# theo2021/OnDA

Measured on AMD Instinct MI355X. Metric: adaptation-step images/sec (fwd+bwd+proto) 512x1024 bs=4, higher is better.
Workload: dtype f32 (f16x2 split emulation); 1 GPU; hybrid_switch adaptation step (step + update_ema), 1024x512, bs=4 per micro-batch, 1 micro-batch(es) per GPU and optimizer step, dynamic branch, DeepLabV2-ResNet50 ProDA head, random-init weights; global_batch=4, parallelism=dp1, branch=dynamic, micro_batches_per_gpu=1, inputs=resident in HBM

## Files before the change

### onda_amd/csrc/conv_l2.hip

```cpp
#include "conv_common.h"

namespace {

typedef _Float16 f16x8 __attribute__((ext_vector_type(8)));
typedef _Float16 f16x2 __attribute__((ext_vector_type(2)));
typedef _Float16 f16x4 __attribute__((ext_vector_type(4)));
typedef float f32x2 __attribute__((ext_vector_type(2)));
typedef unsigned int u32x2 __attribute__((ext_vector_type(2)));
typedef unsigned int u32x4 __attribute__((ext_vector_type(4)));
typedef int i32x4 __attribute__((ext_vector_type(4)));

#define ZZ(i, jj) (((i) & 1) ? 3 - (jj) : (jj))

constexpr float LIMB2_SCALE = ONDA_LIMB2_SCALE, LIMB2_UNSCALE = 1.f / ONDA_LIMB2_SCALE;

#ifndef ONDA_NT_OUT
#define ONDA_NT_OUT 1
#endif
constexpr int NT_AUX = ONDA_NT_OUT ? 2 : 0;
template <class T>
__device__ __forceinline__ void store_out(T* p, T v) {
  if constexpr (ONDA_NT_OUT) __builtin_nontemporal_store(v, p); else *p = v;
}
constexpr unsigned OOB = 0x80000000u;
// ... 29 lines not shown
  const bool ok = (unsigned)hi < (unsigned)c.Hi && (unsigned)wi < (unsigned)c.Wi;
  return ok ? (unsigned)(((p.bH + hi) * c.Wi + wi) * c.ldx) * 4u + chunk16 : 0x80000000u;
}

struct Scale2 {
  float s, inv;
};
__device__ __forceinline__ Scale2 scale_from(float m);
__device__ __forceinline__ Scale2 scale_of(const float* __restrict__ amax) { return scale_from(amax_read(amax)); }
__device__ __forceinline__ Scale2 scale_from(const float m) {
  int e = 0;
  if (m > 0.f && m < 3.0e38f) {
    int ex;
    frexpf(m, &ex);
    e = 15 - ex;
    e = e > 100 ? 100 : (e < -100 ? -100 : e);
  }
  return Scale2{ldexpf(1.f, e), ldexpf(1.f, -e)};
}

__device__ __forceinline__ unsigned cvt2h(float lo, float hi) {
  return __builtin_bit_cast(unsigned, __builtin_convertvector(f32x2{lo, hi}, f16x2));
}
__device__ __forceinline__ f32x2 unpack2h(unsigned p) {
  return __builtin_convertvector(__builtin_bit_cast(f16x2, p), f32x2);
}

__global__ __launch_bounds__(256) void split_h2_kernel(const float* __restrict__ x, long long rows, int C, int ldx,
                                                       _Float16* __restrict__ dst, int ldo, long long plane,
                                                       const float* __restrict__ amax) {
  const float s = scale_of(amax).s;
  const int c8 = C >> 3;
  const long long n = rows * c8;
  for (long long e = (long long)blockIdx.x * 256 + threadIdx.x; e < n; e += (long long)gridDim.x * 256) {
    const long long row = e / c8;
    const int ch = (int)(e - row * c8) * 8;
    const f32x4 v0 = *reinterpret_cast<const f32x4*>(x + row * ldx + ch) * s;
    const f32x4 v1 = *reinterpret_cast<const f32x4*>(x + row * ldx + ch + 4) * s;
    u32x4 l1, l2;
#pragma unroll
    for (int h = 0; h < 4; ++h) {
      const float a = h < 2 ? v0[2 * h] : v1[2 * h - 4], b = h < 2 ? v0[2 * h + 1] : v1[2 * h - 3];
      const unsigned p = cvt2h(a, b);
      const f32x2 f = unpack2h(p);
      l1[h] = p;
      l2[h] = cvt2h((a - f[0]) * LIMB2_SCALE, (b - f[1]) * LIMB2_SCALE);
    }
    _Float16* o = dst + limb_at((size_t)row, ch, ldo);
    *reinterpret_cast<u32x4*>(o) = l1;
    *reinterpret_cast<u32x4*>(o + LIMB2_OFS) = l2;
  }
}

__global__ __launch_bounds__(256) void stem_im2col_l2_kernel(const float* __restrict__ x, _Float16* __restrict__ dst,
                                                             long long plane, int B, int H, int W, int Ho, int Wo, int Kp,
                                                             const float* __restrict__ amax) {
  const float sc = scale_of(amax).s;
  const int k8 = Kp >> 3;
  const long long n = (long long)B * Ho * Wo * k8;
  for (long long e = (long long)blockIdx.x * 256 + threadIdx.x; e < n; e += (long long)gridDim.x * 256) {
    const long long m = e / k8;
    const int k0 = (int)(e - m * k8) * 8;
    const int wo = (int)(m % Wo);
    const long long tq = m / Wo;
    const int ho = (int)(tq % Ho), b = (int)(tq / Ho);
    float v[8];
#pragma unroll
    for (int j = 0; j < 8; ++j) {
      const int k = k0 + j;
      float val = 0.f;
      if (k < 147) {
        const int tap = k / 3, cc = k - tap * 3;
        const int r = tap / 7, t7 = tap - r * 7;
        const int hi = ho * 2 - 3 + r, wi = wo * 2 - 3 + t7;
        if ((unsigned)hi < (unsigned)H && (unsigned)wi < (unsigned)W) val = x[(((size_t)b * 3 + cc) * H + hi) * W + wi];
      }
      v[j] = val * sc;
    }
    u32x4 l1, l2;
#pragma unroll
    for (int h = 0; h < 4; ++h) {
      const unsigned pk = cvt2h(v[2 * h], v[2 * h + 1]);
      const f32x2 f = unpack2h(pk);
      l1[h] = pk;
      l2[h] = cvt2h((v[2 * h] - f[0]) * LIMB2_SCALE, (v[2 * h + 1] - f[1]) * LIMB2_SCALE);
    }
    _Float16* o = dst + limb_at((size_t)m, k0, Kp);
    *reinterpret_cast<u32x4*>(o) = l1;
    *reinterpret_cast<u32x4*>(o + LIMB2_OFS) = l2;
  }
}

#define ONDA_SWAP4(INSN, A, B)                                                                                          \
  asm volatile("s_nop 1\n\t" INSN " %0, %4\n\t" INSN " %1, %5\n\t" INSN " %2, %6\n\t" INSN " %3, %7\n\ts_nop 0"         \
               : "+v"(A[0]), "+v"(A[1]), "+v"(A[2]), "+v"(A[3]), "+v"(B[0]), "+v"(B[1]), "+v"(B[2]), "+v"(B[3]))
__device__ __forceinline__ void rows_reduce4(float& s1, float& s2, float& mn, float& mx) {
#if defined(__HIP_DEVICE_COMPILE__)
  float A[4] = {s1, s2, mn, mx}, B[4] = {s1, s2, mn, mx};
  ONDA_SWAP4("v_permlane16_swap_b32", A, B);
  float C[4] = {A[0] + B[0], A[1] + B[1], fminf(A[2], B[2]), fmaxf(A[3], B[3])};
  float D[4] = {C[0], C[1], C[2], C[3]};
  ONDA_SWAP4("v_permlane32_swap_b32", C, D);
  s1 = C[0] + D[0];
  s2 = C[1] + D[1];
  mn = fminf(C[2], D[2]);
  mx = fmaxf(C[3], D[3]);
#endif
}

template <int WM, int WN, bool COUNTED = false, bool AFFINE = true>
__device__ __forceinline__ void l2_epilogue(const ConvK& a, const f32x4 (&acc)[4][4], unsigned char* scratch, int tile_m, int m0,
                                            int n0, int wm, int wn, int lane, float ua, float ub, unsigned y_bytes = 0) {
  constexpr int BN = 64 * WN, NW = WM * WN, NT = NW * 64;
  constexpr int TRS = 68;
  const OndaConv& c = a.c;
  const int t = threadIdx.x, wave = t >> 6;
  unsigned long long* est = a.stamps != nullptr && t == 0 ? a.stamps + (size_t)blockIdx.x * 32 + 24 : nullptr;
  if (est) est[0] = __builtin_amdgcn_s_memtime();
  float* red = reinterpret_cast<float*>(scratch + NW * (16 * TRS * 4));
  const int SR = a.stats_rows;
  if (a.stats != nullptr) {
#pragma unroll
    for (int jn = 0; jn < 4; ++jn) {
      float s1 = 0.f, s2 = 0.f, mn = 3.0e38f, mxv = -3.0e38f;
#pragma unroll
      for (int i = 0; i < 4; ++i)
#pragma unroll
        for (int e = 0; e < 4; ++e) {
          const float v = acc[i][jn][e];
          s1 += v;
          s2 += v * v;
          mn = fminf(mn, v);
          mxv = fmaxf(mxv, v);
        }
      rows_reduce4(s1, s2, mn, mxv);
      if (lane < 16) {
        const int col = (wn * 4 + jn) * 16 + lane;
        red[(wm * BN + col) * 4 + 0] = (s1 * ua) * ub;
        red[(wm * BN + col) * 4 + 1] = (((s2 * ua) * ub) * ua) * ub;
        red[(wm * BN + col) * 4 + 2] = (mn * ua) * ub;
        red[(wm * BN + col) * 4 + 3] = (mxv * ua) * ub;
      }
// ... 1688 lines not shown
    }
    if (!late && nlive > 0) __builtin_amdgcn_s_barrier();
  }

#pragma unroll
  for (int i = 0; i < 4; ++i)
#pragma unroll
    for (int j = 0; j < 4; ++j) acc[i][j] = ((acc[i][j] + accx[i][j] * LIMB2_UNSCALE) * unscale_a) * unscale_b;
  if (stp) stp[2] = __builtin_amdgcn_s_memtime();
  __syncthreads();
  float* tr = reinterpret_cast<float*>(lds + (t >> 6) * 4096);
  const int cl = (lane & 15) * 4, rl = lane >> 4;
  const int cc = c0 + wn * 64 + cl;
#pragma unroll
  for (int i = 0; i < 4; ++i) {
#pragma unroll
    for (int jn = 0; jn < 4; ++jn)
#pragma unroll
      for (int e = 0; e < 4; ++e) tr[(4 * (lane >> 4) + e) * 64 + jn * 16 + (lane & 15)] = acc[i][jn][e];
    __builtin_amdgcn_wave_barrier();
#pragma unroll
    for (int r = 0; r < 4; ++r) {
      const int row = 4 * r + rl;
      const f32x4 v = *reinterpret_cast<const f32x4*>(tr + row * 64 + cl);
      const int n = n0 + (wm * 4 + i) * 16 + row;
      if (n < c.Cout && cc < c.Cin) *reinterpret_cast<f32x4*>(a.slabs + (((size_t)ks * c.Cout + n) * a.taps + tap) * c.Cin + cc) = v;
    }
    __builtin_amdgcn_wave_barrier();
  }
  if (stp) stp[3] = __builtin_amdgcn_s_memtime();
}

}

extern "C" {

int onda_split_h2(const float* x, int64_t rows, int C, int ldx, void* dst, int ldo, int64_t plane, const float* amax,
                  onda_stream_t s) {
  (void)plane;
  ONDA_REQUIRE(x && dst && amax && rows > 0 && C > 0 && C % 8 == 0 && ldx >= C && ldx % 4 == 0 && ldo >= C && ldo % 32 == 0);
  if (!ONDA_ALIGNED16(x) || !ONDA_ALIGNED16(dst)) return ONDA_EALIGN;
  const long long n = rows * (C / 8);
  const int blocks = (int)(n / 256 / 4 + 1 > 2048 ? 2048 : n / 256 / 4 + 1);
  hipLaunchKernelGGL(split_h2_kernel, dim3(blocks), dim3(256), 0, ONDA_STREAM(s), x, (long long)rows, C, ldx,
                     static_cast<_Float16*>(dst), ldo, (long long)plane, amax);
  return ONDA_LAUNCH_RESULT();
}

int onda_stem_im2col_l2(const float* x_nchw, const float* xamax, void* dst, int64_t plane, int B, int H, int W, int Ho, int Wo,
                        int Kp, onda_stream_t s) {
  (void)plane;
  ONDA_REQUIRE(x_nchw && xamax && dst && Kp % 32 == 0 && Kp >= 147 && B > 0 && Ho > 0 && Wo > 0);
  if (!ONDA_ALIGNED16(dst)) return ONDA_EALIGN;
  const long long n = (long long)B * Ho * Wo * (Kp / 8);
  const int blocks = (int)(n / 256 / 2 + 1 > 4096 ? 4096 : n / 256 / 2 + 1);
  hipLaunchKernelGGL(stem_im2col_l2_kernel, dim3(blocks), dim3(256), 0, ONDA_STREAM(s), x_nchw, static_cast<_Float16*>(dst),
                     (long long)plane, B, H, W, Ho, Wo, Kp, xamax);
  return ONDA_LAUNCH_RESULT();
}

}

namespace {
struct L2Overrides { bool has_variant; int variant; bool short_k128, stationary; int sched; };
L2Overrides l2_overrides() {
  static const int short_k128 = getenv("ONDA_L2_SHORTK128") ? atoi(getenv("ONDA_L2_SHORTK128")) : 1;
  const char* v = getenv("ONDA_L2_VARIANT");
  const char* a = getenv("ONDA_L2_STATIONARY");
  return {v != nullptr, v ? atoi(v) : 0, short_k128 != 0, a != nullptr && atoi(a) != 0, conv_sched_override()};
}

int l2_variant_mc(long long M, int Cout, const L2Overrides& o) {
  if (o.has_variant) return o.variant;
  if (Cout <= 64) return 2;
  const long long t256 = ((M + 255) / 256) * ((Cout + 127) / 128);
  return t256 >= 200 ? 0 : 1;
}

constexpr int L2X_MAX_KSTEPS = 32;

struct L2Epilogue { bool plain; bool dense_out; long long y_total; };

struct L2Plan {
  int kernel, variant, BM, BN, tilesM, tilesN, grid, G, rem, sub, tiles_dp;
  bool balanced;
  int rem_rows() const { return tilesM - (tilesM * tilesN - rem) / tilesN; }
  int stats_rows_total() const { return tilesM + (balanced ? rem_rows() * (sub - 1) : 0); }
};

L2Plan l2_plan(long long M, int Cout, int taps, int Cin, bool have_ws, long long stat_split, bool plain_schedule, const L2Epilogue* epi) {
  const L2Overrides o = l2_overrides();
  const int KT = taps * (Cin / 32);
  L2Plan q;
  q.variant = l2_variant_mc(M, Cout, o);
  if (q.variant == 0 && o.short_k128 && !o.has_variant && (KT <= 8 || (KT <= 16 && Cout >= 512) || (KT <= 32 && Cout >= 2048)))
    q.variant = 1;
  q.BM = q.variant == 1 ? 128 : 256;
  q.BN = q.variant == 2 ? 64 : 128;
  q.tilesM = (int)((M + q.BM - 1) / q.BM);
  q.tilesN = (Cout + q.BN - 1) / q.BN;
  const int cus = conv_resident_workgroups() / 2;
  q.G = q.variant == 0 ? cus : 2 * cus;
  q.sub = q.BM / (256 / (q.BN / 4));
  const int tiles = q.tilesM * q.tilesN;
  q.rem = tiles % q.G;
  const double t_tile_us = 2.0 * q.BM * q.BN * taps * Cin / 1.4e6;
  const double fix_us = 6.0 + (q.G + 2.0 * q.rem) * (q.BM * q.BN / 16384.0) * 0.02;
  q.balanced = have_ws && q.rem != 0 && KT >= 4 && t_tile_us * (1.0 - (double)q.rem / q.G) > fix_us &&
               (size_t)q.G * 2 * q.BM * q.BN <= (size_t)onda_conv_ws_floats() && q.G <= 1024;
// ... 317 lines not shown
```

### onda_amd/csrc/loss_proto.hip

```cpp
#include "common.h"

namespace {

constexpr int KMAX = 32;
constexpr float LOG_CLAMP = -9.21034037f;

__global__ void sum_partials_kernel(const float* __restrict__ ws, int nblocks, int nvals, float scale,
                                    float* __restrict__ result) {
  const int j = threadIdx.x >> 6, lane = threadIdx.x & 63;
  if (j >= nvals) return;
  double s = 0.0;
  for (int b = lane; b < nblocks; b += 64) s += (double)ws[(size_t)b * nvals + j];
  s = wave_sum_d(s);
  if (lane == 0) result[j] = (float)(s * (double)scale);
}

__device__ __forceinline__ float load_row_max(const float* __restrict__ row, int K, float* v) {
  float m = -INFINITY;
#pragma unroll
  for (int k = 0; k < KMAX; ++k)
    if (k < K) {
      v[k] = row[k];
      m = fmaxf(m, v[k]);
    }
// ... 535 lines not shown
          const float x0 = tile[l32 * PA_TS + ch], x1 = tile[l32 * PA_TS + ch + 1];
          a0 += x0 * x0;
          a1 += x1 * x1;
        }
        f2 += a0 + a1;
      }
      const float* ap = tile + l32 * PA_TS + half_lane * 64;
      const float* bp = ph + l32 * PA_PS + half * 128 + half_lane * 64;
#pragma unroll 8
      for (int s_ = 0; s_ < 64; ++s_) acc = __builtin_amdgcn_mfma_f32_32x32x2f32(ap[s_], bp[s_], acc, 0, 0, 0);
      __builtin_amdgcn_wave_barrier();
      if (half == 0) {
        acc_h0 = acc;
#pragma unroll
        for (int v = 0; v < 16; ++v) acc[v] = 0.f;
      }
    }
#pragma unroll
    for (int v = 0; v < 16; ++v) acc[v] += acc_h0[v];
#pragma unroll
    for (int v = 0; v < 16; ++v) tile[(8 * (v >> 2) + 4 * half_lane + (v & 3)) * PA_GS + l32] = acc[v];
    __builtin_amdgcn_wave_barrier();
    const int64_t n = n0 + l32;
    if (half_lane == 0 && n < N) {
      float d[KMAX];
      float dmin = INFINITY;
#pragma unroll
      for (int k = 0; k < KMAX; ++k)
        if (k < K) {
          d[k] = sqrtf(fmaxf(f2 + pn[k] - 2.f * tile[l32 * PA_GS + k], 0.f));
          dmin = fminf(dmin, d[k]);
        }
      const Posterior o = posterior<true>(d, dmin, tau, prior != nullptr, pr_, K);
      if (o.best - o.second < margin || fabsf(o.best - thresh) < margin || !(o.best == o.best)) {
        flagged[atomicAdd(nflagged, 1)] = (int)n;
      } else {
        labels[n] = o.best < thresh ? 255 : o.arg;
        if (soft) {
#pragma unroll
          for (int k = 0; k < KMAX; ++k)
            if (k < K) soft[(size_t)n * K + k] = d[k];
        }
        a_conf += o.conf;
        a_soft += o.best;
        a_prior += o.prmax;
      }
    }
    __builtin_amdgcn_wave_barrier();
  }
  block_sum3(wave_sum(a_conf), wave_sum(a_soft), wave_sum(a_prior), red, ws);
}

constexpr int SUMS_BLOCKS = 256;

__global__ __launch_bounds__(256) void proto_class_sums_kernel(const float* __restrict__ feat, int ldf,
                                                               const int32_t* __restrict__ cls,
                                                               float* __restrict__ ws, int64_t N, int C, int K,
                                                               int64_t rows_per_block) {
  extern __shared__ float acc[];
  float* cnt = acc + (size_t)2 * K * C;
  const int t = threadIdx.x;
  for (int i = t; i < 2 * K * C + K; i += 256) acc[i] = 0.f;
  __syncthreads();
  const int64_t n0 = (int64_t)blockIdx.x * rows_per_block;
  const int64_t n1 = min(N, n0 + rows_per_block);
  for (int64_t n = n0; n < n1; ++n) {
    const int k = cls[n];
    if ((unsigned)k >= (unsigned)K) continue;
    for (int ch = t; ch < C; ch += 256) {
      const float v = feat[(size_t)n * ldf + ch];
      acc[(size_t)k * C + ch] += v;
      acc[(size_t)(K + k) * C + ch] += v * v;
    }
    if (t == 0) cnt[k] += 1.f;
  }
  __syncthreads();
  float* dst = ws + (size_t)blockIdx.x * (2 * K * C + K);
  for (int i = t; i < 2 * K * C + K; i += 256) dst[i] = acc[i];
}

__global__ void proto_sums_finalize_kernel(const float* __restrict__ ws, int nblocks, int KC2, int K,
                                           float* __restrict__ sums, float* __restrict__ counts) {
  const int i = blockIdx.x * blockDim.x + threadIdx.x;
  if (i >= KC2 + K) return;
  float s = 0.f;
  for (int b = 0; b < nblocks; ++b) s += ws[(size_t)b * (KC2 + K) + i];
  if (i < KC2)
    sums[i] = s;
  else
    counts[i - KC2] = s;
}

__global__ void proto_ema_kernel(float* __restrict__ proto, float* __restrict__ sqmean, const float* __restrict__ sums,
                                 const float* __restrict__ counts, float lam, int K, int C) {
  const int i = blockIdx.x * blockDim.x + threadIdx.x;
  if (i >= K * C) return;
  const int k = i / C;
  const float n = counts[k];
  const float keep = n > 0.f ? lam : 1.f;
  const float denom = n > 0.f ? n : 1.f;
  proto[i] = proto[i] * keep + (1.f - keep) * (sums[i] / denom);
  sqmean[i] = sqmean[i] * keep + (1.f - keep) * (sums[(size_t)K * C + i] / denom);
}

__global__ void proto_append_kernel(float* __restrict__ proto, float* __restrict__ sqmean, float* __restrict__ counter,
                                    const float* __restrict__ sums, const float* __restrict__ counts, int K, int C) {
  const int i = blockIdx.x * blockDim.x + threadIdx.x;
  if (i >= K * C) return;
  const int k = i / C;
  const float n = counts[k];
  const float tot = counter[k] + n;
  const float denom = tot > 0.f ? tot : 1.f;
  proto[i] += (sums[i] - proto[i] * n) / denom;
  sqmean[i] += (sums[(size_t)K * C + i] - sqmean[i] * n) / denom;
}
__global__ void proto_append_counter_kernel(float* __restrict__ counter, const float* __restrict__ counts, int K) {
  const int k = threadIdx.x;
  if (k < K) counter[k] += counts[k];
}

constexpr int MT_BLOCK = 4096;
template <class E>
__device__ __forceinline__ int mt_entry_of(const E* __restrict__ table, int n, int block) {
  __shared__ int starts[1024];
  const bool in_lds = n <= 1024;
  if (in_lds) {
    for (int i = threadIdx.x; i < n; i += blockDim.x) starts[i] = table[i].first_block;
    __syncthreads();
  }
  int lo = 0, hi = n - 1;
  while (lo < hi) {
    const int mid = (lo + hi + 1) >> 1;
    if ((in_lds ? starts[mid] : table[mid].first_block) <= block) lo = mid; else hi = mid - 1;
  }
  return lo;
}

template <class E>
__device__ __forceinline__ E mt_block(const E* __restrict__ table, int n_entries, int64_t& i0, int64_t& i1) {
// ... 136 lines not shown
  const int64_t mfma = PA_GRID + PA_LIST_GRID + (N + 4 + 2) / 3;
  return (int)(nb > mfma ? nb : mfma);
}

int onda_proto_assign(const float* feat, int ldf, const float* prior, int ldp, const float* proto, const float* sigma,
                      int mahalanobis, float tau, float thresh, int64_t* labels, float* soft, float* result, float* ws,
                      int64_t N, int C, int K, onda_stream_t s) {
  ONDA_REQUIRE(feat && proto && labels && result && ws && C == 256 && K >= 1 && K <= KMAX && N >= 1 && ldf % 4 == 0);
  ONDA_REQUIRE(!mahalanobis || sigma);
  if (!ONDA_ALIGNED16(feat) || !ONDA_ALIGNED16(proto) || (sigma && !ONDA_ALIGNED16(sigma))) return ONDA_EALIGN;
  if (N >= (1ll << 31)) {
    const int64_t nb = pa_direct_blocks(N);
    hipLaunchKernelGGL(proto_assign_kernel, dim3((unsigned)nb), dim3(256), 0, ONDA_STREAM(s), feat, ldf, prior, ldp, proto, sigma,
                       mahalanobis, tau, thresh, labels, soft, ws, N, K, nullptr, nullptr);
    hipLaunchKernelGGL(sum_partials_kernel, dim3(1), dim3(192), 0, ONDA_STREAM(s), ws, (int)nb, 3, (float)(1.0 / (double)N),
                       result);
    return ONDA_LAUNCH_RESULT();
  }
  int* list = reinterpret_cast<int*>(ws + 3 * (PA_GRID + PA_LIST_GRID));
  int* list_len = list + N;
  hipError_t e = hipMemsetAsync(list_len, 0, sizeof(int), ONDA_STREAM(s));
  if (e != hipSuccess) return (int)e;
  hipLaunchKernelGGL(proto_assign_mfma_kernel, dim3(PA_GRID), dim3(64 * PA_WAVES), 0, ONDA_STREAM(s), feat, ldf, prior, ldp, proto, sigma,
                     mahalanobis, tau, thresh, 1.0e-3f, labels, soft, ws, list, list_len, N, K);
  hipLaunchKernelGGL(proto_assign_kernel, dim3(PA_LIST_GRID), dim3(256), 0, ONDA_STREAM(s), feat, ldf, prior, ldp, proto, sigma,
                     mahalanobis, tau, thresh, labels, soft, ws + 3 * PA_GRID, N, K, list, list_len);
  hipLaunchKernelGGL(sum_partials_kernel, dim3(1), dim3(192), 0, ONDA_STREAM(s), ws, PA_GRID + PA_LIST_GRID, 3,
                     (float)(1.0 / (double)N), result);
  return ONDA_LAUNCH_RESULT();
}

int onda_proto_distances(const float* feat, int ldf, const float* proto, const float* sigma, int mahalanobis, float* dist,
                         int64_t N, int C, int K, onda_stream_t s) {
  ONDA_REQUIRE(feat && proto && dist && N >= 1 && C == 256 && K >= 1 && K <= KMAX && ldf % 4 == 0 && (!mahalanobis || sigma));
  if (!ONDA_ALIGNED16(feat) || !ONDA_ALIGNED16(proto) || (sigma && !ONDA_ALIGNED16(sigma))) return ONDA_EALIGN;
  int64_t nb = (N + 3) / 4;
  if (nb > 4096) nb = 4096;
  hipLaunchKernelGGL(proto_distances_kernel, dim3((unsigned)nb), dim3(256), 0, ONDA_STREAM(s), feat, ldf, proto, sigma, mahalanobis,
                     dist, N, K);
  return ONDA_LAUNCH_RESULT();
}

int64_t onda_proto_sums_ws(int64_t N, int C, int K) { return (int64_t)SUMS_BLOCKS * (2 * K * C + K); }

int onda_proto_class_sums(const float* feat, int ldf, const int32_t* cls, float* sums, float* counts, float* ws,
                          int64_t N, int C, int K, onda_stream_t s) {
  ONDA_REQUIRE(feat && cls && sums && counts && ws && N >= 1);
  const size_t lds = ((size_t)2 * K * C + K) * sizeof(float);
  ONDA_REQUIRE(lds <= 64 * 1024);
  const int64_t rpb = (N + SUMS_BLOCKS - 1) / SUMS_BLOCKS;
  hipLaunchKernelGGL(proto_class_sums_kernel, dim3(SUMS_BLOCKS), dim3(256), lds, ONDA_STREAM(s), feat, ldf, cls, ws, N,
                     C, K, rpb);
  const int tot = 2 * K * C + K;
  hipLaunchKernelGGL(proto_sums_finalize_kernel, dim3((tot + 255) / 256), dim3(256), 0, ONDA_STREAM(s), ws, SUMS_BLOCKS,
                     2 * K * C, K, sums, counts);
  return ONDA_LAUNCH_RESULT();
}

int onda_proto_ema(float* proto, float* sqmean, const float* sums, const float* counts, float lam, int K, int C,
                   onda_stream_t s) {
  ONDA_REQUIRE(proto && sqmean && sums && counts);
  hipLaunchKernelGGL(proto_ema_kernel, dim3((K * C + 255) / 256), dim3(256), 0, ONDA_STREAM(s), proto, sqmean, sums,
                     counts, lam, K, C);
  return ONDA_LAUNCH_RESULT();
}

int onda_proto_append(float* proto, float* sqmean, float* counter, const float* sums, const float* counts, int K, int C,
                      onda_stream_t s) {
  ONDA_REQUIRE(proto && sqmean && counter && sums && counts && K <= 64);
  hipLaunchKernelGGL(proto_append_kernel, dim3((K * C + 255) / 256), dim3(256), 0, ONDA_STREAM(s), proto, sqmean,
                     counter, sums, counts, K, C);
  hipLaunchKernelGGL(proto_append_counter_kernel, dim3(1), dim3(64), 0, ONDA_STREAM(s), counter, counts, K);
  return ONDA_LAUNCH_RESULT();
}

int onda_sgd_multi(const OndaSgdEntry* table, int n, float momentum, float weight_decay, float grad_scale, int64_t max_n,
                   onda_stream_t s) {
  ONDA_REQUIRE(table && n >= 1 && max_n >= 1 && max_n < (1ll << 31));
  hipLaunchKernelGGL(sgd_multi_kernel, dim3((unsigned)max_n), dim3(256), 0, ONDA_STREAM(s), table, n, momentum, weight_decay, grad_scale);
  return ONDA_LAUNCH_RESULT();
}

int onda_multi_tensor_block(void) { return MT_BLOCK; }

int onda_ema_multi(const OndaEmaEntry* table, int n, int64_t max_n, onda_stream_t s) {
  ONDA_REQUIRE(table && n >= 1 && max_n >= 1 && max_n < (1ll << 31));
  hipLaunchKernelGGL(ema_multi_kernel, dim3((unsigned)max_n), dim3(256), 0, ONDA_STREAM(s), table, n);
  return ONDA_LAUNCH_RESULT();
}

#ifndef ONDA_SRC_HASH
#define ONDA_SRC_HASH "unknown"
#endif
float onda_limb2_scale(void) { return ONDA_LIMB2_SCALE; }

const char* onda_version(void) { return "onda_hip 0.2 (gfx950) src=" ONDA_SRC_HASH; }

}
```

### onda_amd/csrc/pointwise.hip

```cpp
#include "common.h"
#include <type_traits>

namespace {

#define LD4(p) (*reinterpret_cast<const f32x4*>(p))

typedef _Float16 mp_f16x2 __attribute__((ext_vector_type(2)));
typedef float mp_f32x2 __attribute__((ext_vector_type(2)));
typedef unsigned mp_u32x2 __attribute__((ext_vector_type(2)));
__global__ __launch_bounds__(256) void maxpool_fwd_kernel(const float* __restrict__ x, float* __restrict__ y,
                                                          uint8_t* __restrict__ idx, int B, int Hi, int Wi, int C,
                                                          int Ho, int Wo, _Float16* __restrict__ yl,
                                                          const float* __restrict__ amax) {
  const int c4 = C / 4;
  float so = 1.f;
  if (yl != nullptr) {
    const float m = amax_read(amax);
    int ex = 0;
    if (m > 0.f && m < 3.0e38f) {
      frexpf(m, &ex);
      ex = 15 - ex;
      ex = ex > 100 ? 100 : (ex < -100 ? -100 : ex);
    }
    so = ldexpf(1.f, ex);
  }
  const size_t total = (size_t)B * Ho * Wo * c4;
  for (size_t e = (size_t)blockIdx.x * blockDim.x + threadIdx.x; e < total; e += (size_t)gridDim.x * blockDim.x) {
    const int col = (int)(e % c4) * 4;
    size_t q = e / c4;
    const int wo = (int)(q % Wo);
    q /= Wo;
    const int ho = (int)(q % Ho), b = (int)(q / Ho);
    f32x4 best = {-INFINITY, -INFINITY, -INFINITY, -INFINITY};
    int slot[4] = {0, 0, 0, 0};
    bool first = true;
    for (int r = 0; r < 3; ++r) {
      const int hi = ho * 2 - 1 + r;
      if ((unsigned)hi >= (unsigned)Hi) continue;
      for (int s = 0; s < 3; ++s) {
        const int wi = wo * 2 - 1 + s;
        if ((unsigned)wi >= (unsigned)Wi) continue;
        const f32x4 v = LD4(x + (((size_t)b * Hi + hi) * Wi + wi) * C + col);
#pragma unroll
        for (int j = 0; j < 4; ++j) {
          if (first || v[j] > best[j] || v[j] != v[j]) {
            best[j] = v[j];
            slot[j] = r * 3 + s;
          }
        }
        first = false;
      }
    }
    if (yl != nullptr) {
      const f32x4 w = best * so;
      mp_u32x2 l1, l2;
#pragma unroll
      for (int h = 0; h < 2; ++h) {
        const mp_f16x2 p = __builtin_convertvector(mp_f32x2{w[2 * h], w[2 * h + 1]}, mp_f16x2);
        const mp_f32x2 f = __builtin_convertvector(p, mp_f32x2);
        l1[h] = __builtin_bit_cast(unsigned, p);
        l2[h] = __builtin_bit_cast(unsigned, __builtin_convertvector(mp_f32x2{(w[2 * h] - f[0]) * ONDA_LIMB2_SCALE, (w[2 * h + 1] - f[1]) * ONDA_LIMB2_SCALE}, mp_f16x2));
      }
      _Float16* o = yl + limb_at(e / c4, col, C);
      *reinterpret_cast<mp_u32x2*>(o) = l1;
      *reinterpret_cast<mp_u32x2*>(o + LIMB2_OFS) = l2;
    } else {
      *reinterpret_cast<f32x4*>(y + e * 4) = best;
    }
    *reinterpret_cast<uint32_t*>(idx + e * 4) =
        (uint32_t)slot[0] | ((uint32_t)slot[1] << 8) | ((uint32_t)slot[2] << 16) | ((uint32_t)slot[3] << 24);
  }
}

__global__ __launch_bounds__(256) void maxpool_bwd_kernel(const float* __restrict__ dy, const uint8_t* __restrict__ idx,
                                                          float* __restrict__ dx, int B, int Hi, int Wi, int C, int Ho,
                                                          int Wo) {
  const int c4 = C / 4;
  const size_t total = (size_t)B * Hi * Wi * c4;
  for (size_t e = (size_t)blockIdx.x * blockDim.x + threadIdx.x; e < total; e += (size_t)gridDim.x * blockDim.x) {
    const int col = (int)(e % c4) * 4;
    size_t q = e / c4;
    const int wi = (int)(q % Wi);
    q /= Wi;
    const int hi = (int)(q % Hi), b = (int)(q / Hi);
    f32x4 acc = {0.f, 0.f, 0.f, 0.f};
    const int ho_lo = hi / 2, ho_hi = (hi + 1) / 2;
    const int wo_lo = wi / 2, wo_hi = (wi + 1) / 2;
    for (int ho = ho_lo; ho <= ho_hi; ++ho) {
      if (ho >= Ho) continue;
      for (int wo = wo_lo; wo <= wo_hi; ++wo) {
        if (wo >= Wo) continue;
        const int slot = (hi - (ho * 2 - 1)) * 3 + (wi - (wo * 2 - 1));
        const size_t o = (((size_t)b * Ho + ho) * Wo + wo) * C + col;
        const uint32_t pk = *reinterpret_cast<const uint32_t*>(idx + o);
        const f32x4 g = LD4(dy + o);
#pragma unroll
        for (int j = 0; j < 4; ++j)
          if ((int)((pk >> (8 * j)) & 0xff) == slot) acc[j] += g[j];
      }
    }
    *reinterpret_cast<f32x4*>(dx + e * 4) = acc;
  }
}

__global__ __launch_bounds__(256) void se_fc1_kernel(const float* __restrict__ pooled, const float* __restrict__ w1,
                                                     const float* __restrict__ b1, float* __restrict__ hidden, int C, int R) {
  const int b = blockIdx.y, lane = threadIdx.x & 63, r = blockIdx.x * 4 + (threadIdx.x >> 6);
  if (r >= R) return;
  const float* p = pooled + (size_t)b * C;
  float s = 0.f;
  for (int ch = lane; ch < C; ch += 64) s += w1[(size_t)r * C + ch] * p[ch];
  s = wave_sum(s);
  if (lane == 0) hidden[(size_t)b * R + r] = fmaxf(s + b1[r], 0.f);
}

__global__ __launch_bounds__(256) void se_fc2_kernel(const float* __restrict__ hidden, const float* __restrict__ w2,
                                                     const float* __restrict__ b2, float* __restrict__ gate, int C, int R) {
  extern __shared__ float hid[];
  const int b = blockIdx.y, t = threadIdx.x;
  for (int r = t; r < R; r += 256) hid[r] = hidden[(size_t)b * R + r];
  __syncthreads();
  const int ch = blockIdx.x * 256 + t;
  if (ch >= C) return;
  float s = b2[ch];
  for (int r = 0; r < R; ++r) s += w2[(size_t)ch * R + r] * hid[r];
  gate[(size_t)b * C + ch] = 1.f / (1.f + expf(-s));
}

__global__ void se_bwd_w2_kernel(const float* __restrict__ dgate, const float* __restrict__ gate,
                                 const float* __restrict__ hidden, float* __restrict__ dw2, float* __restrict__ db2,
                                 int B, int C, int R) {
  const int i = blockIdx.x * blockDim.x + threadIdx.x;
  if (i >= C * R) return;
  const int ch = i / R, r = i % R;
  float s = 0.f, sb = 0.f;
  for (int b = 0; b < B; ++b) {
    const float g = gate[(size_t)b * C + ch];
    const float d = dgate[(size_t)b * C + ch] * g * (1.f - g);
    s += d * hidden[(size_t)b * R + r];
    sb += d;
  }
  dw2[i] = s;
  if (r == 0) db2[ch] = sb;
}

__global__ __launch_bounds__(256) void se_bwd_hidden_kernel(const float* __restrict__ dgate,
                                                            const float* __restrict__ gate,
                                                            const float* __restrict__ hidden,
                                                            const float* __restrict__ w2, float* __restrict__ dpre1,
                                                            int C, int R) {
  const int b = blockIdx.x, t = threadIdx.x, lane = t & 63, wave = t >> 6;
  for (int r = wave; r < R; r += 4) {
    float s = 0.f;
    for (int ch = lane; ch < C; ch += 64) {
      const float g = gate[(size_t)b * C + ch];
      s += dgate[(size_t)b * C + ch] * g * (1.f - g) * w2[(size_t)ch * R + r];
    }
    s = wave_sum(s);
    if (lane == 0) dpre1[(size_t)b * R + r] = hidden[(size_t)b * R + r] > 0.f ? s : 0.f;
  }
}

__global__ void se_bwd_w1_kernel(const float* __restrict__ dpre1, const float* __restrict__ pooled,
                                 const float* __restrict__ w1, float* __restrict__ dw1, float* __restrict__ db1,
                                 float* __restrict__ dpooled, int B, int C, int R, float scale) {
  const int i = blockIdx.x * blockDim.x + threadIdx.x;
  if (i < R * C) {
    const int r = i / C, ch = i % C;
    float s = 0.f, sb = 0.f;
    for (int b = 0; b < B; ++b) {
      s += dpre1[(size_t)b * R + r] * pooled[(size_t)b * C + ch];
      sb += dpre1[(size_t)b * R + r];
    }
    dw1[i] = s;
    if (ch == 0) db1[r] = sb;
  }
  if (i < B * C) {
    const int b = i / C, ch = i % C;
    float s = 0.f;
    for (int r = 0; r < R; ++r) s += dpre1[(size_t)b * R + r] * w1[(size_t)r * C + ch];
    dpooled[i] = s * scale;
  }
}

__global__ __launch_bounds__(256) void chan_scale_kernel(const float* __restrict__ x, const float* __restrict__ gate,
                                                         const float* __restrict__ add, float* __restrict__ out,
                                                         int64_t HW, int C, size_t total4) {
  const int c4 = C / 4;
  for (size_t e = (size_t)blockIdx.x * blockDim.x + threadIdx.x; e < total4; e += (size_t)gridDim.x * blockDim.x) {
    const int col = (int)(e % c4) * 4;
    const int b = (int)((e / c4) / HW);
    f32x4 v = LD4(x + e * 4) * LD4(gate + (size_t)b * C + col);
    if (add) v += LD4(add + (size_t)b * C + col);
    *reinterpret_cast<f32x4*>(out + e * 4) = v;
  }
}

struct Lerp {
  int i0, i1;
  float l0, l1;
};
__device__ __forceinline__ Lerp lerp_index(int dst, float scale, int in_size) {
#pragma clang fp contract(off)
  const float src = scale * (float)dst;
  Lerp o;
  o.i0 = (int)src;
  o.i1 = o.i0 + (o.i0 < in_size - 1 ? 1 : 0);
  o.l1 = src - (float)o.i0;
  o.l0 = 1.f - o.l1;
  return o;
}

struct Pixel {
// ... 538 lines not shown
}

template <class Grad>
int upsample_bwd_two_pass(const Grad& grad, const float* logits, int ldl, float* dlogits, float* ws, int B, int h, int w, int K,
                          int H, int W, onda_stream_t s) {
  const float sy = ac_scale(h, H), sx = ac_scale(w, W);
  const int CW = uce_block_cols(w, W);
  ONDA_REQUIRE(CW >= 1);
  const size_t lds = ((size_t)(CW + 2) * K + (size_t)UCE_SPAN * K + 2 * UCE_SPAN) * sizeof(float);
  ONDA_REQUIRE(lds <= 160 * 1024);
  if (lds > 64 * 1024) {
    static size_t granted = 0;
    if (lds > granted) {
      const hipError_t e = hipFuncSetAttribute(reinterpret_cast<const void*>(upsample_bwd_rows_kernel<Grad>),
                                               hipFuncAttributeMaxDynamicSharedMemorySize, (int)lds);
      if (e != hipSuccess) return (int)e;
      granted = lds;
    }
  }
  hipLaunchKernelGGL(upsample_bwd_rows_kernel<Grad>, dim3((w + CW - 1) / CW, B * H), dim3(256), lds, ONDA_STREAM(s), grad, logits, ldl,
                     ws, B, h, w, K, H, W, sy, sx, 1.f / sx, CW);
  hipLaunchKernelGGL(upsample_ce_bwd_cols_kernel, dim3(ew_grid((size_t)B * h * w * ldl)), dim3(256), 0, ONDA_STREAM(s), ws, dlogits,
                     ldl, B, h, w, K, H, sy, 1.f / sy);
  return ONDA_LAUNCH_RESULT();
}

}

extern "C" {

int onda_maxpool_fwd(const float* x, float* y, uint8_t* idx, int B, int Hi, int Wi, int C, int Ho, int Wo,
                     onda_stream_t s) {
  ONDA_REQUIRE(x && y && idx && C % 4 == 0);
  const size_t total = (size_t)B * Ho * Wo * (C / 4);
  hipLaunchKernelGGL(maxpool_fwd_kernel, dim3(ew_grid(total)), dim3(256), 0, ONDA_STREAM(s), x, y, idx, B, Hi, Wi, C, Ho,
                     Wo, static_cast<_Float16*>(nullptr), static_cast<const float*>(nullptr));
  return ONDA_LAUNCH_RESULT();
}

int onda_maxpool_fwd_limbs(const float* x, const float* xamax, void* yl, uint8_t* idx, int B, int Hi, int Wi, int C, int Ho, int Wo,
                           onda_stream_t s) {
  ONDA_REQUIRE(x && xamax && yl && idx && C % 32 == 0);
  if (!ONDA_ALIGNED16(yl)) return ONDA_EALIGN;
  const size_t total = (size_t)B * Ho * Wo * (C / 4);
  hipLaunchKernelGGL(maxpool_fwd_kernel, dim3(ew_grid(total)), dim3(256), 0, ONDA_STREAM(s), x, static_cast<float*>(nullptr), idx, B,
                     Hi, Wi, C, Ho, Wo, static_cast<_Float16*>(yl), xamax);
  return ONDA_LAUNCH_RESULT();
}

int onda_maxpool_bwd(const float* dy, const uint8_t* idx, float* dx, int B, int Hi, int Wi, int C, int Ho, int Wo,
                     onda_stream_t s) {
  ONDA_REQUIRE(dy && dx && idx && C % 4 == 0);
  const size_t total = (size_t)B * Hi * Wi * (C / 4);
  hipLaunchKernelGGL(maxpool_bwd_kernel, dim3(ew_grid(total)), dim3(256), 0, ONDA_STREAM(s), dy, idx, dx, B, Hi, Wi, C,
                     Ho, Wo);
  return ONDA_LAUNCH_RESULT();
}

int onda_se_fc_fwd(const float* pooled, const float* w1, const float* b1, const float* w2, const float* b2,
                   float* hidden, float* gate, int B, int C, int R, onda_stream_t s) {
  ONDA_REQUIRE(pooled && w1 && b1 && w2 && b2 && hidden && gate && R <= 4096);
  hipLaunchKernelGGL(se_fc1_kernel, dim3((R + 3) / 4, B), dim3(256), 0, ONDA_STREAM(s), pooled, w1, b1, hidden, C, R);
  hipLaunchKernelGGL(se_fc2_kernel, dim3((C + 255) / 256, B), dim3(256), R * sizeof(float), ONDA_STREAM(s), hidden, w2, b2, gate, C,
                     R);
  return ONDA_LAUNCH_RESULT();
}

int onda_se_fc_bwd(const float* dgate, const float* pooled, const float* hidden, const float* gate, const float* w1,
                   const float* w2, float* dw1, float* db1, float* dw2, float* db2, float* dpooled, float* ws,
                   float dpooled_scale, int B, int C, int R, onda_stream_t s) {
  ONDA_REQUIRE(dgate && pooled && hidden && gate && w1 && w2 && dw1 && db1 && dw2 && db2 && dpooled && ws);
  hipLaunchKernelGGL(se_bwd_w2_kernel, dim3((C * R + 255) / 256), dim3(256), 0, ONDA_STREAM(s), dgate, gate, hidden, dw2,
                     db2, B, C, R);
  hipLaunchKernelGGL(se_bwd_hidden_kernel, dim3(B), dim3(256), 0, ONDA_STREAM(s), dgate, gate, hidden, w2, ws, C, R);
  const int n = (R > B ? R : B) * C;
  hipLaunchKernelGGL(se_bwd_w1_kernel, dim3((n + 255) / 256), dim3(256), 0, ONDA_STREAM(s), ws, pooled, w1, dw1, db1,
                     dpooled, B, C, R, dpooled_scale);
  return ONDA_LAUNCH_RESULT();
}

int onda_chan_scale(const float* x, const float* gate, const float* add, float* out, int B, int64_t HW, int C,
                    onda_stream_t s) {
  ONDA_REQUIRE(x && gate && out && C % 4 == 0);
  const size_t total4 = (size_t)B * HW * C / 4;
  hipLaunchKernelGGL(chan_scale_kernel, dim3(ew_grid(total4)), dim3(256), 0, ONDA_STREAM(s), x, gate, add, out, HW, C,
                     total4);
  return ONDA_LAUNCH_RESULT();
}

int onda_upsample_fwd(const float* logits, int ldl, float* out, int B, int h, int w, int K, int H, int W,
                      onda_stream_t s) {
  ONDA_REQUIRE(logits && out && K <= ldl);
  hipLaunchKernelGGL((upsample_kernel<false>), dim3(ew_grid((size_t)B * H * W)), dim3(256), 0, ONDA_STREAM(s), logits,
                     ldl, out, (uint8_t*)nullptr, (const uint8_t*)nullptr, (unsigned long long*)nullptr, B, h, w, K, H, W,
                     ac_scale(h, H), ac_scale(w, W));
  return ONDA_LAUNCH_RESULT();
}

int onda_upsample_argmax(const float* logits, int ldl, uint8_t* cls, int B, int h, int w, int K, int H, int W,
                         onda_stream_t s) {
  ONDA_REQUIRE(logits && cls && K <= ldl && K <= 255);
  hipLaunchKernelGGL((upsample_kernel<true>), dim3(ew_grid((size_t)B * H * W)), dim3(256), 0, ONDA_STREAM(s), logits,
                     ldl, (float*)nullptr, cls, (const uint8_t*)nullptr, (unsigned long long*)nullptr, B, h, w, K, H, W,
                     ac_scale(h, H), ac_scale(w, W));
  return ONDA_LAUNCH_RESULT();
}

int onda_upsample_argmax_hist(const float* logits, int ldl, const uint8_t* labels, int64_t* hist, uint8_t* cls, int B,
                              int h, int w, int K, int H, int W, onda_stream_t s) {
  ONDA_REQUIRE(logits && labels && hist && K <= ldl && K <= 255);
  unsigned grid = ew_grid((size_t)B * H * W);
  if (K * K <= UPS_HIST_LDS && grid > 1024u) grid = 1024u;
  hipLaunchKernelGGL((upsample_kernel<true>), dim3(grid), dim3(256), 0, ONDA_STREAM(s), logits,
                     ldl, (float*)nullptr, cls, labels, reinterpret_cast<unsigned long long*>(hist), B, h, w, K, H, W,
                     ac_scale(h, H), ac_scale(w, W));
  return ONDA_LAUNCH_RESULT();
}

int onda_ece_bins_local(void) { return ECE_BINS_LDS; }

int onda_upsample_ece(const float* rows, int ld, const uint8_t* labels, int64_t* table, int bins, int probs, int64_t* hist, int B,
                      int h, int w, int K, int H, int W, onda_stream_t s) {
  ONDA_REQUIRE(rows && labels && table && K >= 1 && K <= ld && K <= 255 && bins >= 1 && bins <= (1 << 20) && B >= 1 && h >= 1 &&
               w >= 1 && H >= 1 && W >= 1);
  if (!ONDA_ALIGNED16(table) || (hist && !ONDA_ALIGNED16(hist))) return ONDA_EALIGN;
  const size_t total = (size_t)B * H * W;
  const int local = bins <= ECE_BINS_LDS;
// ... 79 lines not shown
```

Measured before the change: 42.96 images/s.

## Tile stem im2col through LDS, batch proto sums loads, unroll maxpool/SE backward

Several unrelated kernel changes ship together. The stem im2col now stages a 21-row input patch in shared memory per output-row tile and pairs limb stores across lanes so each lane writes a full line. Proto class sums and finalize batch their loads ahead to expose memory-level parallelism. Maxpool backward issues all four window loads unconditionally, with 32-bit indexing when the range allows, and SE hidden backward spreads rows across more blocks. Together these target redundant gathers and latency-bound serial loops, at the cost of more shared memory and registers and a fixed grid shape for the stem kernel.

Result: no change. 43.15 images/s, median of 6 (+0.4%).

```diff
diff --git a/onda_amd/csrc/conv_l2.hip b/onda_amd/csrc/conv_l2.hip
--- a/onda_amd/csrc/conv_l2.hip
+++ b/onda_amd/csrc/conv_l2.hip
@@ -105,30 +105,64 @@
   }
 }
 
+__device__ __forceinline__ void store_limb_lines(_Float16* o, u32x4 l1, u32x4 l2, bool whole) {
+  if (!whole) {
+    *reinterpret_cast<u32x4*>(o) = l1;
+    *reinterpret_cast<u32x4*>(o + LIMB2_OFS) = l2;
+    return;
+  }
+  const bool hi = (threadIdx.x & 4) != 0;
+  const u32x4 send = hi ? l1 : l2;
+  u32x4 recv;
+#pragma unroll
+  for (int j = 0; j < 4; ++j) recv[j] = (unsigned)__shfl_xor((int)send[j], 4, 64);
+  const unsigned long long mine = reinterpret_cast<unsigned long long>(o);
+  const unsigned long long partner = ((unsigned long long)(unsigned)__shfl_xor((int)(mine >> 32), 4, 64) << 32) |
+                                     (unsigned)__shfl_xor((int)(unsigned)mine, 4, 64);
+  _Float16* po = reinterpret_cast<_Float16*>(partner);
+  _Float16* a1 = hi ? po + LIMB2_OFS : o;
+  _Float16* a2 = hi ? o + LIMB2_OFS : po;
+  *reinterpret_cast<u32x4*>(a1) = hi ? recv : l1;
+  *reinterpret_cast<u32x4*>(a2) = hi ? l2 : recv;
+}
+
+constexpr int STEM_TW = 64, STEM_PW = 2 * STEM_TW + 5;
 __global__ __launch_bounds__(256) void stem_im2col_l2_kernel(const float* __restrict__ x, _Float16* __restrict__ dst,
                                                              long long plane, int B, int H, int W, int Ho, int Wo, int Kp,
                                                              const float* __restrict__ amax) {
+  __shared__ float patch[21 * STEM_PW];
   const float sc = scale_of(amax).s;
+  const int t = threadIdx.x;
+  const int tiles_w = (Wo + STEM_TW - 1) / STEM_TW;
+  const int wt = blockIdx.x % tiles_w, q = blockIdx.x / tiles_w;
+  const int ho = q % Ho, b = q / Ho;
+  const int wo0 = wt * STEM_TW, tw = min(STEM_TW, Wo - wo0);
+  for (int i = t; i < 21 * STEM_PW; i += 256) {
+    const int seg = i / STEM_PW, p = i - seg * STEM_PW;
+    const int cc = seg / 7, r = seg - cc * 7;
+    const int hi = ho * 2 - 3 + r, wi = wo0 * 2 - 3 + p;
+    float val = 0.f;
+    if ((unsigned)hi < (unsigned)H && (unsigned)wi < (unsigned)W) val = x[(((size_t)b * 3 + cc) * H + hi) * W + wi];
+    patch[i] = val * sc;
+  }
+  __syncthreads();
   const int k8 = Kp >> 3;
-  const long long n = (long long)B * Ho * Wo * k8;
-  for (long long e = (long long)blockIdx.x * 256 + threadIdx.x; e < n; e += (long long)gridDim.x * 256) {
-    const long long m = e / k8;
-    const int k0 = (int)(e - m * k8) * 8;
-    const int wo = (int)(m % Wo);
-    const long long tq = m / Wo;
-    const int ho = (int)(tq % Ho), b = (int)(tq / Ho);
+  const size_t m0 = ((size_t)b * Ho + ho) * Wo + wo0;
+  for (int it = t; it < tw * k8; it += 256) {
+    const int ml = it / k8, k0 = (it - ml * k8) * 8;
+    int tap = k0 / 3, cc = k0 - tap * 3;
+    int r = tap / 7, t7 = tap - r * 7;
     float v[8];
 #pragma unroll
     for (int j = 0; j < 8; ++j) {
-      const int k = k0 + j;
-      float val = 0.f;
-      if (k < 147) {
-        const int tap = k / 3, cc = k - tap * 3;
-        const int r = tap / 7, t7 = tap - r * 7;
-        const int hi = ho * 2 - 3 + r, wi = wo * 2 - 3 + t7;
-        if ((unsigned)hi < (unsigned)H && (unsigned)wi < (unsigned)W) val = x[(((size_t)b * 3 + cc) * H + hi) * W + wi];
-      }
-      v[j] = val * sc;
+      v[j] = r < 7 ? patch[(cc * 7 + r) * STEM_PW + 2 * ml + t7] : 0.f;
+      if (++cc == 3) {
+        cc = 0;
+        if (++t7 == 7) {
+          t7 = 0;
+          ++r;
+        }
+      }
     }
     u32x4 l1, l2;
 #pragma unroll
@@ -138,9 +172,7 @@
       l1[h] = pk;
       l2[h] = cvt2h((v[2 * h] - f[0]) * LIMB2_SCALE, (v[2 * h + 1] - f[1]) * LIMB2_SCALE);
     }
-    _Float16* o = dst + limb_at((size_t)m, k0, Kp);
-    *reinterpret_cast<u32x4*>(o) = l1;
-    *reinterpret_cast<u32x4*>(o + LIMB2_OFS) = l2;
+    store_limb_lines(dst + limb_at(m0 + ml, k0, Kp), l1, l2, __ballot(1) == ~0ull);
   }
 }
 
@@ -1935,9 +1967,9 @@
   (void)plane;
   ONDA_REQUIRE(x_nchw && xamax && dst && Kp % 32 == 0 && Kp >= 147 && B > 0 && Ho > 0 && Wo > 0);
   if (!ONDA_ALIGNED16(dst)) return ONDA_EALIGN;
-  const long long n = (long long)B * Ho * Wo * (Kp / 8);
-  const int blocks = (int)(n / 256 / 2 + 1 > 4096 ? 4096 : n / 256 / 2 + 1);
-  hipLaunchKernelGGL(stem_im2col_l2_kernel, dim3(blocks), dim3(256), 0, ONDA_STREAM(s), x_nchw, static_cast<_Float16*>(dst),
+  const long long blocks = (long long)B * Ho * ((Wo + STEM_TW - 1) / STEM_TW);
+  ONDA_REQUIRE(blocks < (1ll << 31));
+  hipLaunchKernelGGL(stem_im2col_l2_kernel, dim3((unsigned)blocks), dim3(256), 0, ONDA_STREAM(s), x_nchw, static_cast<_Float16*>(dst),
                      (long long)plane, B, H, W, Ho, Wo, Kp, xamax);
   return ONDA_LAUNCH_RESULT();
 }
diff --git a/onda_amd/csrc/loss_proto.hip b/onda_amd/csrc/loss_proto.hip
--- a/onda_amd/csrc/loss_proto.hip
+++ b/onda_amd/csrc/loss_proto.hip
@@ -611,6 +611,8 @@
 }
 
 constexpr int SUMS_BLOCKS = 256;
+constexpr int SUMS_AHEAD = 8;
+constexpr int FIN_AHEAD = 16;
 
 __global__ __launch_bounds__(256) void proto_class_sums_kernel(const float* __restrict__ feat, int ldf,
                                                                const int32_t* __restrict__ cls,
@@ -623,15 +625,27 @@
   __syncthreads();
   const int64_t n0 = (int64_t)blockIdx.x * rows_per_block;
   const int64_t n1 = min(N, n0 + rows_per_block);
-  for (int64_t n = n0; n < n1; ++n) {
-    const int k = cls[n];
-    if ((unsigned)k >= (unsigned)K) continue;
+  for (int64_t n = n0; n < n1; n += SUMS_AHEAD) {
+    int kk[SUMS_AHEAD];
+#pragma unroll
+    for (int u = 0; u < SUMS_AHEAD; ++u) kk[u] = n + u < n1 ? cls[n + u] : -1;
     for (int ch = t; ch < C; ch += 256) {
-      const float v = feat[(size_t)n * ldf + ch];
-      acc[(size_t)k * C + ch] += v;
-      acc[(size_t)(K + k) * C + ch] += v * v;
-    }
-    if (t == 0) cnt[k] += 1.f;
+      float v[SUMS_AHEAD];
+#pragma unroll
+      for (int u = 0; u < SUMS_AHEAD; ++u) v[u] = feat[(size_t)min(n + u, n1 - 1) * ldf + ch];
+#pragma unroll
+      for (int u = 0; u < SUMS_AHEAD; ++u) {
+        const int k = kk[u];
+        if ((unsigned)k >= (unsigned)K) continue;
+        acc[(size_t)k * C + ch] += v[u];
+        acc[(size_t)(K + k) * C + ch] += v[u] * v[u];
+      }
+    }
+    if (t == 0) {
+#pragma unroll
+      for (int u = 0; u < SUMS_AHEAD; ++u)
+        if ((unsigned)kk[u] < (unsigned)K) cnt[kk[u]] += 1.f;
+    }
   }
   __syncthreads();
   float* dst = ws + (size_t)blockIdx.x * (2 * K * C + K);
@@ -643,7 +657,14 @@
   const int i = blockIdx.x * blockDim.x + threadIdx.x;
   if (i >= KC2 + K) return;
   float s = 0.f;
-  for (int b = 0; b < nblocks; ++b) s += ws[(size_t)b * (KC2 + K) + i];
+  for (int b = 0; b < nblocks; b += FIN_AHEAD) {
+    float v[FIN_AHEAD];
+#pragma unroll
+    for (int u = 0; u < FIN_AHEAD; ++u) v[u] = ws[(size_t)min(b + u, nblocks - 1) * (KC2 + K) + i];
+#pragma unroll
+    for (int u = 0; u < FIN_AHEAD; ++u)
+      if (b + u < nblocks) s += v[u];
+  }
   if (i < KC2)
     sums[i] = s;
   else
@@ -886,7 +907,7 @@
   hipLaunchKernelGGL(proto_class_sums_kernel, dim3(SUMS_BLOCKS), dim3(256), lds, ONDA_STREAM(s), feat, ldf, cls, ws, N,
                      C, K, rpb);
   const int tot = 2 * K * C + K;
-  hipLaunchKernelGGL(proto_sums_finalize_kernel, dim3((tot + 255) / 256), dim3(256), 0, ONDA_STREAM(s), ws, SUMS_BLOCKS,
+  hipLaunchKernelGGL(proto_sums_finalize_kernel, dim3((tot + 63) / 64), dim3(64), 0, ONDA_STREAM(s), ws, SUMS_BLOCKS,
                      2 * K * C, K, sums, counts);
   return ONDA_LAUNCH_RESULT();
 }
diff --git a/onda_amd/csrc/pointwise.hip b/onda_amd/csrc/pointwise.hip
--- a/onda_amd/csrc/pointwise.hip
+++ b/onda_amd/csrc/pointwise.hip
@@ -72,34 +72,42 @@
   }
 }
 
+template <class I>
 __global__ __launch_bounds__(256) void maxpool_bwd_kernel(const float* __restrict__ dy, const uint8_t* __restrict__ idx,
                                                           float* __restrict__ dx, int B, int Hi, int Wi, int C, int Ho,
                                                           int Wo) {
-  const int c4 = C / 4;
-  const size_t total = (size_t)B * Hi * Wi * c4;
-  for (size_t e = (size_t)blockIdx.x * blockDim.x + threadIdx.x; e < total; e += (size_t)gridDim.x * blockDim.x) {
-    const int col = (int)(e % c4) * 4;
-    size_t q = e / c4;
-    const int wi = (int)(q % Wi);
-    q /= Wi;
-    const int hi = (int)(q % Hi), b = (int)(q / Hi);
+  const unsigned c4 = (unsigned)C / 4;
+  const I total = (I)B * Hi * Wi * c4;
+  for (I e = (I)blockIdx.x * blockDim.x + threadIdx.x; e < total; e += (I)gridDim.x * blockDim.x) {
+    const I q0 = e / c4;
+    const int col = (int)(e - q0 * c4) * 4;
+    const I q1 = q0 / (unsigned)Wi;
+    const int wi = (int)(q0 - q1 * (unsigned)Wi);
+    const int b = (int)(q1 / (unsigned)Hi), hi = (int)(q1 - (I)b * (unsigned)Hi);
+    const int ho2[2] = {hi / 2, (hi + 1) / 2};
+    const int wo2[2] = {wi / 2, (wi + 1) / 2};
+    uint32_t pk[4];
+    f32x4 g[4];
+    bool ok[4];
+    int slot[4];
+#pragma unroll
+    for (int w = 0; w < 4; ++w) {
+      const int ho = ho2[w >> 1], wo = wo2[w & 1];
+      ok[w] = ((w >> 1) == 0 || ho2[1] != ho2[0]) && ((w & 1) == 0 || wo2[1] != wo2[0]) && ho < Ho && wo < Wo;
+      slot[w] = (hi - (ho * 2 - 1)) * 3 + (wi - (wo * 2 - 1));
+      const size_t o = (((size_t)b * Ho + min(ho, Ho - 1)) * Wo + min(wo, Wo - 1)) * C + col;
+      pk[w] = *reinterpret_cast<const uint32_t*>(idx + o);
+      g[w] = LD4(dy + o);
+    }
     f32x4 acc = {0.f, 0.f, 0.f, 0.f};
-    const int ho_lo = hi / 2, ho_hi = (hi + 1) / 2;
-    const int wo_lo = wi / 2, wo_hi = (wi + 1) / 2;
-    for (int ho = ho_lo; ho <= ho_hi; ++ho) {
-      if (ho >= Ho) continue;
-      for (int wo = wo_lo; wo <= wo_hi; ++wo) {
-        if (wo >= Wo) continue;
-        const int slot = (hi - (ho * 2 - 1)) * 3 + (wi - (wo * 2 - 1));
-        const size_t o = (((size_t)b * Ho + ho) * Wo + wo) * C + col;
-        const uint32_t pk = *reinterpret_cast<const uint32_t*>(idx + o);
-        const f32x4 g = LD4(dy + o);
-#pragma unroll
-        for (int j = 0; j < 4; ++j)
-          if ((int)((pk >> (8 * j)) & 0xff) == slot) acc[j] += g[j];
-      }
-    }
-    *reinterpret_cast<f32x4*>(dx + e * 4) = acc;
+#pragma unroll
+    for (int w = 0; w < 4; ++w) {
+      if (!ok[w]) continue;
+#pragma unroll
+      for (int j = 0; j < 4; ++j)
+        if ((int)((pk[w] >> (8 * j)) & 0xff) == slot[w]) acc[j] += g[w][j];
+    }
+    *reinterpret_cast<f32x4*>(dx + (size_t)e * 4) = acc;
   }
 }
 
@@ -149,16 +157,16 @@
                                                             const float* __restrict__ hidden,
                                                             const float* __restrict__ w2, float* __restrict__ dpre1,
                                                             int C, int R) {
-  const int b = blockIdx.x, t = threadIdx.x, lane = t & 63, wave = t >> 6;
-  for (int r = wave; r < R; r += 4) {
-    float s = 0.f;
-    for (int ch = lane; ch < C; ch += 64) {
-      const float g = gate[(size_t)b * C + ch];
-      s += dgate[(size_t)b * C + ch] * g * (1.f - g) * w2[(size_t)ch * R + r];
-    }
-    s = wave_sum(s);
-    if (lane == 0) dpre1[(size_t)b * R + r] = hidden[(size_t)b * R + r] > 0.f ? s : 0.f;
-  }
+  const int b = blockIdx.y, lane = threadIdx.x & 63, r = blockIdx.x * 4 + (threadIdx.x >> 6);
+  if (r >= R) return;
+  float s = 0.f;
+#pragma unroll 4
+  for (int ch = lane; ch < C; ch += 64) {
+    const float g = gate[(size_t)b * C + ch];
+    s += dgate[(size_t)b * C + ch] * g * (1.f - g) * w2[(size_t)ch * R + r];
+  }
+  s = wave_sum(s);
+  if (lane == 0) dpre1[(size_t)b * R + r] = hidden[(size_t)b * R + r] > 0.f ? s : 0.f;
 }
 
 __global__ void se_bwd_w1_kernel(const float* __restrict__ dpre1, const float* __restrict__ pooled,
@@ -803,8 +811,12 @@
                      onda_stream_t s) {
   ONDA_REQUIRE(dy && dx && idx && C % 4 == 0);
   const size_t total = (size_t)B * Hi * Wi * (C / 4);
-  hipLaunchKernelGGL(maxpool_bwd_kernel, dim3(ew_grid(total)), dim3(256), 0, ONDA_STREAM(s), dy, idx, dx, B, Hi, Wi, C,
-                     Ho, Wo);
+  const unsigned blocks = ew_grid(total);
+  if (total + (size_t)blocks * 256 < 0xFFFFFFFFull)
+    hipLaunchKernelGGL(maxpool_bwd_kernel<unsigned>, dim3(blocks), dim3(256), 0, ONDA_STREAM(s), dy, idx, dx, B, Hi, Wi, C, Ho, Wo);
+  else
+    hipLaunchKernelGGL(maxpool_bwd_kernel<unsigned long long>, dim3(blocks), dim3(256), 0, ONDA_STREAM(s), dy, idx, dx, B, Hi, Wi,
+                       C, Ho, Wo);
   return ONDA_LAUNCH_RESULT();
 }
 
@@ -823,7 +835,7 @@
   ONDA_REQUIRE(dgate && pooled && hidden && gate && w1 && w2 && dw1 && db1 && dw2 && db2 && dpooled && ws);
   hipLaunchKernelGGL(se_bwd_w2_kernel, dim3((C * R + 255) / 256), dim3(256), 0, ONDA_STREAM(s), dgate, gate, hidden, dw2,
                      db2, B, C, R);
-  hipLaunchKernelGGL(se_bwd_hidden_kernel, dim3(B), dim3(256), 0, ONDA_STREAM(s), dgate, gate, hidden, w2, ws, C, R);
+  hipLaunchKernelGGL(se_bwd_hidden_kernel, dim3((R + 3) / 4, B), dim3(256), 0, ONDA_STREAM(s), dgate, gate, hidden, w2, ws, C, R);
   const int n = (R > B ? R : B) * C;
   hipLaunchKernelGGL(se_bwd_w1_kernel, dim3((n + 255) / 256), dim3(256), 0, ONDA_STREAM(s), ws, pooled, w1, dw1, db1,
                      dpooled, B, C, R, dpooled_scale);
```
